# HoangGiang93/mujoco_sim

Measured on AMD Instinct MI355X. Metric: env-steps/sec (whole node) at 4096 envs, 24-DoF/30-contact scene; 1/2/4/8 GPUs, higher is better.
Workload: dtype f32

## Files before the change

mujoco_sim_amd/build.py:

```python
import os
import subprocess
import sys

HERE = os.path.dirname(os.path.abspath(__file__))
CSRC = os.path.join(HERE, "csrc")
OBJ = os.path.join(HERE, "build")
LIB = os.path.join(HERE, "libmjhip.so")
API = os.path.join("..", "..", "include", "mjhip.h")
KERNEL_HEADERS = ["step_kernel.h", "patch_pgs.h", "window_pgs.h", "dev_math.h", "dev_collide.h", "dev_convex.h", "dev_types.h"]
DENSE_HEADERS = ["dense_pgs.h"] + KERNEL_HEADERS
WINDOW_HEADERS = ["window_kernel.h", "step_kernel.h", "patch_pgs.h", "window_pgs.h", "dev_math.h", "dev_collide.h", "dev_convex.h", "dev_types.h"]
SOURCES = {
    "engine.hip": KERNEL_HEADERS + ["dev_ray.h", "ray_bvh.h", "dev_depth.h", "dev_scan.h", "dev_heightscan.h", "dev_render.h", "dev_light.h", "dev_texture.h", "ray_tables.h", API],
    "window.hip": WINDOW_HEADERS + [API],
    "dense.hip": DENSE_HEADERS + [API],
    "hfield.hip": KERNEL_HEADERS + [API],
    "ray.hip": ["dev_ray.h", "ray_bvh.h", API],
    "depth.hip": ["dev_depth.h", "dev_ray.h", "ray_bvh.h", API],
    "scan.hip": ["dev_scan.h", "dev_depth.h", "dev_ray.h", "ray_bvh.h", API],
    "heightscan.hip": ["dev_heightscan.h", "dev_scan.h", "dev_depth.h", "dev_ray.h", "ray_bvh.h", API],
    "render.hip": ["dev_render.h", "dev_depth.h", "dev_ray.h", "ray_bvh.h", API],
    "light.hip": ["dev_light.h", "dev_render.h", "dev_depth.h", "dev_ray.h", "ray_bvh.h", API],
    "texture.hip": ["dev_texture.h", "dev_render.h", "dev_depth.h", "dev_ray.h", "ray_bvh.h", API],
    "group.hip": ["host_pool.h", API],
    "model_builder.cpp": ["hmath.h", API],
    "scenes.cpp": ["hmath.h", API],
    "host_sim.cpp": ["host_sim.h", API],
    "mjcf_loader.cpp": ["hmath.h", API],
}
FLAGS = ["--offload-arch=gfx950", "-O3", "-std=c++17", "-fPIC", "-munsafe-fp-atomics", "-fno-slp-vectorize", "-Wno-unused-result"]
SOURCE_FLAGS = {"window.hip": ["-mllvm", "-pragma-unroll-threshold=200000"]}
FLAGS += os.environ.get("MJH_EXTRA_FLAGS", "").split()
if os.environ.get("MJH_BUILD_DIR"):
    OBJ = os.environ["MJH_BUILD_DIR"]; LIB = os.path.join(OBJ, "libmjhip.so")


def _digest(paths, extra=""):
    import hashlib
    h = hashlib.sha256(extra.encode())
    for p in paths:
        if os.path.exists(p):
            with open(p, "rb") as f:
                h.update(f.read())
    return h.hexdigest()


def build(force=False, verbose=False):
    hipcc = os.environ.get("HIPCC", "/opt/rocm/bin/hipcc")
    os.makedirs(OBJ, exist_ok=True)
    objs, digests, stale = [], [], []
    for src, deps in SOURCES.items():
        sp = os.path.join(CSRC, src)
        if not os.path.exists(sp):
            continue
        op = os.path.join(OBJ, os.path.splitext(src)[0] + ".o")
        sflags = FLAGS + SOURCE_FLAGS.get(src, [])
        dg = _digest([sp] + [os.path.join(CSRC, d) for d in deps], " ".join(sflags))
        stamp = op + ".sha256"
        have = open(stamp).read().strip() if os.path.exists(stamp) else ""
        if force or not os.path.exists(op) or have != dg:
            stale.append(([hipcc] + sflags + ["-c", sp, "-o", op], stamp, dg))
        objs.append(op); digests.append(dg)
    link_dg = _digest([], " ".join(digests))
    link_stamp = os.path.join(OBJ, "libmjhip.sha256")
    have = open(link_stamp).read().strip() if os.path.exists(link_stamp) else ""
    if not force and os.path.exists(LIB) and have == link_dg:
        return LIB
    from concurrent.futures import ThreadPoolExecutor

    def _compile(job):
        cmd, stamp, dg = job
        if verbose:
            print(" ".join(cmd), file=sys.stderr)
        subprocess.check_call(cmd)
        with open(stamp, "w") as f:
            f.write(dg)
    with ThreadPoolExecutor(max_workers=max(1, min(4, len(stale)))) as pool:
        for r in [pool.submit(_compile, j) for j in stale]:
            r.result()
    if force or not os.path.exists(LIB) or have != link_dg:
        cmd = [hipcc, "--offload-arch=gfx950", "-shared", "-fPIC"] + objs + ["-ldl", "-o", LIB]
        if verbose:
            print(" ".join(cmd), file=sys.stderr)
        subprocess.check_call(cmd)
# ... 15 lines not shown
```

mujoco_sim_amd/csrc/window_kernel.h:

```cpp
#pragma once
#include "step_kernel.h"

#ifdef WN_PROF_CLK
#define WN_STAT0(x) min((int)(((long long)__builtin_amdgcn_s_memtime() - wn_t0) >> 5) + 1, (1 << 22) - 1)
#else
#define WN_STAT0(x) (x)
#endif

#ifdef MJH_ASM_PROBE
#define WN_STATS(env, ncon, nefc, niter) S.stats[4 * env + 1] = nefc
#else
#define WN_STATS(env, ncon, nefc, niter) S.stats[4 * env] = WN_STAT0(ncon); S.stats[4 * env + 1] = nefc; S.stats[4 * env + 2] = niter
#endif

#ifdef WN_PROF_CLK
__shared__ long long wn_t0;
#endif

#define WN_BC8(M) M(0) M(1) M(2) M(3) M(4) M(5) M(6) M(7)
template <int NV> struct WnWin { float J[NV]; float4 A0, A1, A2, A3; float aref, R, nw, half; };

#define WN_ROR2(d, s0, s1, r0, m0, r1, m1) "v_add_f32_dpp " d ", " s0 ", " s0 " row_ror:" #r0 " row_mask:0xf bank_mask:" #m0 "\n\tv_add_f32_dpp " d ", " s1 ", " s1 " row_ror:" #r1 " row_mask:0xf bank_mask:" #m1 "\n\t"
DEV float wn_fold_tail(const float* z) {
  const int q = threadIdx.x & 15;
  const bool b1 = (q & 2) != 0, b0 = (q & 1) != 0;
  float w[2];
#pragma unroll
  for (int k = 0; k < 2; k++) {
    const float s = b1 ? z[k + 2] : z[k], o = b1 ? z[k] : z[k + 2];
    w[k] = s + __builtin_bit_cast(float, __builtin_amdgcn_update_dpp(0, __builtin_bit_cast(int, o), 0x4E, 0xf, 0xf, true));
  }
  const float s = b0 ? w[1] : w[0], o = b0 ? w[0] : w[1];
  return s + __builtin_bit_cast(float, __builtin_amdgcn_update_dpp(0, __builtin_bit_cast(int, o), 0xB1, 0xf, 0xf, true));
}
DEV void wn_fold_8to4(const float* y, float* z) {
  asm volatile(WN_ROR2("%0", "%4", "%8", 12, 0x5, 4, 0xa) WN_ROR2("%1", "%5", "%9", 12, 0x5, 4, 0xa) WN_ROR2("%2", "%6", "%10", 12, 0x5, 4, 0xa) WN_ROR2("%3", "%7", "%11", 12, 0x5, 4, 0xa)
               : "=&v"(z[0]), "=&v"(z[1]), "=&v"(z[2]), "=&v"(z[3]) : "v"(y[0]), "v"(y[1]), "v"(y[2]), "v"(y[3]), "v"(y[4]), "v"(y[5]), "v"(y[6]), "v"(y[7]));
}
DEV float wn_fold16(const float* x) {
  float y[8], z[4];
  asm volatile("s_nop 1\n\t"
               WN_ROR2("%0", "%8", "%16", 8, 0x3, 8, 0xc) WN_ROR2("%1", "%9", "%17", 8, 0x3, 8, 0xc) WN_ROR2("%2", "%10", "%18", 8, 0x3, 8, 0xc) WN_ROR2("%3", "%11", "%19", 8, 0x3, 8, 0xc)
               WN_ROR2("%4", "%12", "%20", 8, 0x3, 8, 0xc) WN_ROR2("%5", "%13", "%21", 8, 0x3, 8, 0xc) WN_ROR2("%6", "%14", "%22", 8, 0x3, 8, 0xc) WN_ROR2("%7", "%15", "%23", 8, 0x3, 8, 0xc)
               : "=&v"(y[0]), "=&v"(y[1]), "=&v"(y[2]), "=&v"(y[3]), "=&v"(y[4]), "=&v"(y[5]), "=&v"(y[6]), "=&v"(y[7])
               : "v"(x[0]), "v"(x[1]), "v"(x[2]), "v"(x[3]), "v"(x[4]), "v"(x[5]), "v"(x[6]), "v"(x[7]),
                 "v"(x[8]), "v"(x[9]), "v"(x[10]), "v"(x[11]), "v"(x[12]), "v"(x[13]), "v"(x[14]), "v"(x[15]));
  wn_fold_8to4(y, z);
  return wn_fold_tail(z);
}
#define WN_FOLD24_BODY \
    WN_ROR2("%[ya0]", "%[x16]", "%[x20]", 8, 0x3, 8, 0xc) WN_ROR2("%[ya1]", "%[x17]", "%[x21]", 8, 0x3, 8, 0xc) WN_ROR2("%[ya2]", "%[x18]", "%[x22]", 8, 0x3, 8, 0xc) WN_ROR2("%[ya3]", "%[x19]", "%[x23]", 8, 0x3, 8, 0xc) \
    WN_ROR2("%[ya0]", "%[ya0]", "%[ya2]", 12, 0x5, 4, 0xa) WN_ROR2("%[ya1]", "%[ya1]", "%[ya3]", 12, 0x5, 4, 0xa) \
    "v_cndmask_b32_e64 %[t0], %[z2], %[z0], %[m1]\n\t" "v_cndmask_b32_e64 %[t1], %[z3], %[z1], %[m1]\n\t" "v_cndmask_b32_e64 %[t2], %[z0], %[z2], %[m1]\n\t" \
    "v_cndmask_b32_e64 %[t3], %[z1], %[z3], %[m1]\n\t" "v_cndmask_b32_e64 %[ya2], %[ya1], %[ya0], %[m1]\n\t" "v_cndmask_b32_e64 %[ya3], %[ya0], %[ya1], %[m1]\n\t"
// ... 195 lines not shown
  if (dl_lane && q < M.njnt) {
    const int qadr = jnt_qposadr[q], da = jnt_dofadr[q];
    float p[7];
#pragma unroll
    for (int k = 0; k < 7; k++) p[k] = bad ? S.initial_qpos[qrow + qadr + k] : wb[WN_QPOS + qadr + k];
    const float* v = s_v32[es] + da;
    p[0] += h * v[0]; p[1] += h * v[1]; p[2] += h * v[2];
    float w3[3] = {v[3], v[4], v[5]};
    quat_integrate(p + 3, w3, h);
#pragma unroll
    for (int k = 0; k < 7; k++) { S.qpos[qrow + qadr + k] = p[k]; s_qp32[es][qadr + k] = p[k]; }
  }
  if (has_odom) {
    __syncthreads();
    if (dl_lane && q == 0) wn_odom(M, S, env, s_qp32[es], S.qvel + vrow);
  }
  if (dl_lane && q == 0) {
    S.time[env] += M.timestep_d;
    const int cost_hint = wn_cost_hint(M, nwin16, niter);
    WN_STATS(env, wh[1], wh[2], niter);
    S.stats[4 * env + 3] = ((S.stats[4 * env + 3] | flags) & 0xff) | (cost_hint << 8);
  }
}

DEV void wn_run32(const DConst* __restrict__ C, const DState& S, const int env0, const int nenv, const int xflags, const int blk) {
  const DModel& M = C->M;
  constexpr int NV = 24;
  const int lane = threadIdx.x, es = lane >> 5, hq = (lane >> 4) & 1, q = lane & 15;
  const int slot = blk * 2 + es;
  const bool have = slot < nenv;
  const int env = have ? (S.env_order ? S.env_order[env0 + slot] : env0 + slot) : 0;
  float* const wb = S.wbuf + (size_t)env * (size_t)S.wstride;
  const int* const wh = (const int*)wb;
  const int nrow = (have && wh[4] == 1) ? wh[0] : 0;
  if (__ballot(nrow > 0) == 0ull) return;
  const bool mine = nrow > 0;
  const int nwin16 = (nrow + 15) >> 4, nwin = (nrow + 31) >> 5;
  const int nwmax = max(__builtin_amdgcn_readlane(nwin, 0), __builtin_amdgcn_readlane(nwin, 32));
  const int nv = M.nv;
  const int dhi = 16 + (q >> 1);
  const bool lo_on = q < nv, hi_on = dhi < nv;
  const float as_lo = lo_on ? wb[WN_AS + q] : 0.0f, as_hi = hi_on ? wb[WN_AS + dhi] : 0.0f;
  const float ws_lo = lo_on ? wb[WN_AWS + q] : 0.0f, ws_hi = hi_on ? wb[WN_AWS + dhi] : 0.0f;
  WnWin32 win[WN32_NW];
  float f[WN32_NW];
  const float* rows = wb + WN_ROWS + q;
#pragma unroll
  for (int w = 0; w < WN32_NW; w++) if (w < nwmax) {
    WnWin32& W = win[w];
    const bool ok = (2 * w + hq) < nwin16;
    wn_load_row<NV>(rows + (2 * w + hq) * WN_NK * 16, ok, W.J, W.aref, W.R);
    float acc[16], acx[16], Jx[NV];
#pragma unroll
    for (int sidx = 0; sidx < 16; sidx++) { acc[sidx] = 0.0f; acx[sidx] = 0.0f; }
#pragma unroll
    for (int k = 0; k < NV; k++) Jx[k] = WN_SWZ16(W.J[k]);
#pragma unroll
    for (int k = 0; k < NV; k++) asm volatile("" : "+v"(W.J[k]), "+v"(Jx[k]));
    asm volatile("s_nop 1");
#define WN_ACC(sidx) PP_FMAC_BC(acc[sidx], W.J[k], W.J[k], sidx); PP_FMAC_BC(acx[sidx], Jx[k], W.J[k], sidx);
#pragma unroll
    for (int k = 0; k < NV; k++) { PP_BC16(WN_ACC) }
#undef WN_ACC
    float diag = 0.0f;
#pragma unroll
    for (int k = 0; k < NV; k++) diag += W.J[k] * W.J[k];
    const float ARqq = diag + W.R;
    const float inv = ARqq < MJ_MINVAL ? 0.0f : 1.0f / ARqq, ninv = -inv, cinv = hq ? ninv : 0.0f;
    W.nw = ninv; W.half = 0.5f * ARqq;
    W.A0 = make_float4(0 < q ? ninv * acc[0] : 0.0f, 1 < q ? ninv * acc[1] : 0.0f, 2 < q ? ninv * acc[2] : 0.0f, 3 < q ? ninv * acc[3] : 0.0f);
    W.A1 = make_float4(4 < q ? ninv * acc[4] : 0.0f, 5 < q ? ninv * acc[5] : 0.0f, 6 < q ? ninv * acc[6] : 0.0f, 7 < q ? ninv * acc[7] : 0.0f);
    W.A2 = make_float4(8 < q ? ninv * acc[8] : 0.0f, 9 < q ? ninv * acc[9] : 0.0f, 10 < q ? ninv * acc[10] : 0.0f, 11 < q ? ninv * acc[11] : 0.0f);
    W.A3 = make_float4(12 < q ? ninv * acc[12] : 0.0f, 13 < q ? ninv * acc[13] : 0.0f, 14 < q ? ninv * acc[14] : 0.0f, 0.0f);
    W.C0 = make_float4(cinv * acx[0], cinv * acx[1], cinv * acx[2], cinv * acx[3]);
    W.C1 = make_float4(cinv * acx[4], cinv * acx[5], cinv * acx[6], cinv * acx[7]);
    W.C2 = make_float4(cinv * acx[8], cinv * acx[9], cinv * acx[10], cinv * acx[11]);
    W.C3 = make_float4(cinv * acx[12], cinv * acx[13], cinv * acx[14], cinv * acx[15]);
  }
  auto rowsum_i32 = [&](int v) __attribute__((always_inline)) { v = wn_rowsum_i(v); return v + __builtin_amdgcn_ds_swizzle(v, 0x401F); };
  auto rowsum_f32 = [&](float v) __attribute__((always_inline)) { v = wn_rowsum_f(v); return v + WN_SWZ16(v); };
#define WN32_FOR_WINDOWS(...) do { _Pragma("unroll") for (int w = 0; w < WN32_NW; w++) if (w < nwmax) { WnWin32& W = win[w]; float& fw = f[w]; __VA_ARGS__ } } while (0)
  float a_lo = as_lo, a_hi = as_hi;
#pragma unroll
  for (int w = 0; w < WN32_NW; w++) f[w] = 0.0f;
  if (!(M.disableflags & MJH_DSBL_WARMSTART)) {
    float da_lo = 0.0f, da_hi = 0.0f;
    WN32_FOR_WINDOWS({
      const float jar = wn_dot<NV>(W.J, ws_lo, ws_hi) - W.aref;
      fw = (jar < 0.0f && W.R > 0.0f) ? -jar / W.R : 0.0f;
      wn_jt32(W.J, fw, da_lo, da_hi);
    });
    float cost = 0.0f;
    WN32_FOR_WINDOWS({
      const float jda = wn_dot<NV>(W.J, da_lo, da_hi), bb = wn_dot<NV>(W.J, as_lo, as_hi) - W.aref;
      cost += fw * (0.5f * (jda + W.R * fw) + bb);
    });
    cost = rowsum_f32(cost);
    if (cost > 0.0f) {
#pragma unroll
      for (int w = 0; w < WN32_NW; w++) f[w] = 0.0f;
    } else { a_lo += da_lo; a_hi += da_hi; }
  }
  const ImpQ iq = imp_quantum(1.0f / (M.meaninertia * (float)(nv > 1 ? nv : 1)), M.tolerance);
  const int itmax = M.iterations;
  int niter = 0;
  bool act = nrow > 0;
  while (__ballot(act) != 0ull) {
    if (act) {
      int impl = 0;
      WN32_FOR_WINDOWS({
        const float u = wn_dot<NV, false>(W.J, a_lo, a_hi);
        const float fo = fw;
        float tt = ((u - W.aref) + W.R * fo) * W.nw;
        const float nf = -fo;
        float dl;
        WN_ROWS4M(0, 1, 2, 3, W.A0, 0x5); WN_ROWS4M(4, 5, 6, 7, W.A1, 0x5); WN_ROWS4M(8, 9, 10, 11, W.A2, 0x5); WN_ROWS4M(12, 13, 14, 15, W.A3, 0x5);
// ... 106 lines not shown
    WN64_CHAIN16F(W.A, 16, 0x2, 0, 0xc, dx0);                    \
    WN64_BCAST_X1(W.A, 16, 0x4);                                 \
    dx1 = dy; \
    WN64_CHAIN16F(W.A, 32, 0x4, 16, 0x8, dx1);                   \
    WN64_BCAST_X2(W.A, 32, 0x8); \
    WN64_CHAIN16(W.A, 48, 0x8); \
    impl += imp_fixed((W.half * dl) * (2.0f * tt - dl), iq.qs); \
    fw = fo + dl; \
    wn_jt64(W.J, dl, a_lo, a_hi); } while (0)
#ifndef WN_FILL64
#define WN_FILL64 1
#endif
#if WN_FILL64
#define WN64_SWEEP(W, fw) WN64_SWEEP_F(W, fw)
#else
#define WN64_SWEEP(W, fw) WN64_SWEEP_X(W, fw, W.A, 0, 16, 32, 48, (void)0, (void)0, (void)0, (void)0)
#endif

template <int N64W, int N64T> DEV void wn_run64(const DConst* __restrict__ C, const DState& S, const int env0, const int nenv, const int xflags, const int blk, float* const lds64) {
  const DModel& M = C->M;
  constexpr int NV = 24;
  const int lane = threadIdx.x, g = lane >> 4, q = lane & 15;
  const bool have = blk < nenv;
  const int env = have ? (S.env_order ? S.env_order[env0 + blk] : env0 + blk) : 0;
  float* const wb = S.wbuf + (size_t)env * (size_t)S.wstride;
  const int* const wh = (const int*)wb;
  const int nrow = (have && wh[4] == 2) ? wh[0] : 0;
  if (nrow <= 0) return;
  const int nwin16 = (nrow + 15) >> 4, nwin = (nrow + 63) >> 6;
  const int nv = M.nv;
  const int dhi = 16 + (q >> 1);
  const bool lo_on = q < nv, hi_on = dhi < nv;
  const float as_lo = lo_on ? wb[WN_AS + q] : 0.0f, as_hi = hi_on ? wb[WN_AS + dhi] : 0.0f;
  const float ws_lo = lo_on ? wb[WN_AWS + q] : 0.0f, ws_hi = hi_on ? wb[WN_AWS + dhi] : 0.0f;
  WnWin64 win[N64W];
  float f[N64W];
  const float* rows = wb + WN_ROWS + q;
#pragma unroll
  for (int w = 0; w < N64W; w++) if (w < nwin) {
    WnWin64& W = win[w];
    const bool ok = (4 * w + g) < nwin16;
    wn_load_row<NV>(rows + (4 * w + g) * WN_NK * 16, ok, W.J, W.aref, W.R);
    float diag = 0.0f;
#pragma unroll
    for (int k = 0; k < NV; k++) diag += W.J[k] * W.J[k];
    const float ARqq = diag + W.R;
    const float inv = ARqq < MJ_MINVAL ? 0.0f : 1.0f / ARqq, ninv = -inv;
    W.nw = ninv; W.half = 0.5f * ARqq;
#pragma unroll
    for (int G = 0; G < 4; G++) {
      float Jg[NV], acc[16];
#pragma unroll
      for (int k = 0; k < NV; k++) Jg[k] = __builtin_bit_cast(float, __builtin_amdgcn_ds_bpermute((16 * G + q) << 2, __builtin_bit_cast(int, W.J[k])));
#pragma unroll
      for (int sidx = 0; sidx < 16; sidx++) acc[sidx] = 0.0f;
#pragma unroll
      for (int k = 0; k < NV; k++) asm volatile("" : "+v"(W.J[k]), "+v"(Jg[k]));
      asm volatile("s_nop 1");
#define WN_ACC(sidx) PP_FMAC_BC(acc[sidx], Jg[k], W.J[k], sidx);
#pragma unroll
      for (int k = 0; k < NV; k++) { PP_BC16(WN_ACC) }
#undef WN_ACC
#pragma unroll
      for (int sidx = 0; sidx < 16; sidx++) W.A[16 * G + sidx] = (16 * G + sidx) < lane ? ninv * acc[sidx] : 0.0f;
    }
  }
  struct WnTail { float J[NV]; float aref, R, nw, half; };
  WnTail TLS[N64T > 0 ? N64T : 1];
  float ftl[N64T > 0 ? N64T : 1];
  float* const tile = lds64 + lane * 4;
#pragma unroll
  for (int t = 0; t < N64T; t++) {
    ftl[t] = 0.0f;
    if (N64W + t < nwin) {
    WnTail& TL = TLS[t];
    const bool ok = (4 * (N64W + t) + g) < nwin16;
    wn_load_row<NV>(rows + (4 * (N64W + t) + g) * WN_NK * 16, ok, TL.J, TL.aref, TL.R);
    float diag = 0.0f;
#pragma unroll
    for (int k = 0; k < NV; k++) diag += TL.J[k] * TL.J[k];
    const float ARqq = diag + TL.R;
    const float inv = ARqq < MJ_MINVAL ? 0.0f : 1.0f / ARqq, ninv = -inv;
    TL.nw = ninv; TL.half = 0.5f * ARqq;
#pragma unroll
    for (int G = 0; G < 4; G++) {
      float Jg[NV], acc[16];
#pragma unroll
      for (int k = 0; k < NV; k++) Jg[k] = __builtin_bit_cast(float, __builtin_amdgcn_ds_bpermute((16 * G + q) << 2, __builtin_bit_cast(int, TL.J[k])));
#pragma unroll
      for (int sidx = 0; sidx < 16; sidx++) acc[sidx] = 0.0f;
#pragma unroll
      for (int k = 0; k < NV; k++) asm volatile("" : "+v"(TL.J[k]), "+v"(Jg[k]));
      asm volatile("s_nop 1");
#define WN_ACC(sidx) PP_FMAC_BC(acc[sidx], Jg[k], TL.J[k], sidx);
#pragma unroll
      for (int k = 0; k < NV; k++) { PP_BC16(WN_ACC) }
#undef WN_ACC
#pragma unroll
      for (int c4 = 0; c4 < 4; c4++) {
        const int r0 = 16 * G + 4 * c4;
        *(float4*)(tile + t * 4096 + (r0 >> 2) * 256) = make_float4(r0 < lane ? ninv * acc[4 * c4] : 0.0f, r0 + 1 < lane ? ninv * acc[4 * c4 + 1] : 0.0f,
                                                                    r0 + 2 < lane ? ninv * acc[4 * c4 + 2] : 0.0f, r0 + 3 < lane ? ninv * acc[4 * c4 + 3] : 0.0f);
      }
    }
    }
  }
  float T[16];
#define WN64_TLOAD(t, gb) do { const float* tp_ = tile + (t) * 4096 + (4 * (gb)) * 256; \
    const float4 t0_ = *(const float4*)(tp_), t1_ = *(const float4*)(tp_ + 256), t2_ = *(const float4*)(tp_ + 512), t3_ = *(const float4*)(tp_ + 768); \
    T[0] = t0_.x; T[1] = t0_.y; T[2] = t0_.z; T[3] = t0_.w; T[4] = t1_.x; T[5] = t1_.y; T[6] = t1_.z; T[7] = t1_.w; \
    T[8] = t2_.x; T[9] = t2_.y; T[10] = t2_.z; T[11] = t2_.w; T[12] = t3_.x; T[13] = t3_.y; T[14] = t3_.z; T[15] = t3_.w; } while (0)
#define WN64_FOR_TAILS(...) do { _Pragma("unroll") for (int t = 0; t < N64T; t++) if (N64W + t < nwin) { WnTail& TL = TLS[t]; float& ft = ftl[t]; __VA_ARGS__ } } while (0)
  float a_lo = as_lo, a_hi = as_hi;
#pragma unroll
  for (int w = 0; w < N64W; w++) f[w] = 0.0f;
#define WN64_FOR_WINDOWS(...) do { _Pragma("unroll") for (int w = 0; w < N64W; w++) if (w < nwin) { WnWin64& W = win[w]; float& fw = f[w]; __VA_ARGS__ } } while (0)
  if (!(M.disableflags & MJH_DSBL_WARMSTART)) {
    float da_lo = 0.0f, da_hi = 0.0f;
    WN64_FOR_WINDOWS({
      const float jar = wn_dot<NV>(W.J, ws_lo, ws_hi) - W.aref;
      fw = (jar < 0.0f && W.R > 0.0f) ? -jar / W.R : 0.0f;
      wn_jt64(W.J, fw, da_lo, da_hi);
    });
    WN64_FOR_TAILS({
      const float jar = wn_dot<NV>(TL.J, ws_lo, ws_hi) - TL.aref;
      ft = (jar < 0.0f && TL.R > 0.0f) ? -jar / TL.R : 0.0f;
      wn_jt64(TL.J, ft, da_lo, da_hi);
    });
    float cost = 0.0f;
    WN64_FOR_WINDOWS({
      const float jda = wn_dot<NV>(W.J, da_lo, da_hi), bb = wn_dot<NV>(W.J, as_lo, as_hi) - W.aref;
      cost += fw * (0.5f * (jda + W.R * fw) + bb);
    });
    WN64_FOR_TAILS({
      const float jda = wn_dot<NV>(TL.J, da_lo, da_hi), bb = wn_dot<NV>(TL.J, as_lo, as_hi) - TL.aref;
      cost += ft * (0.5f * (jda + TL.R * ft) + bb);
    });
    float dummy = 0.0f;
    cost = wn_rowsum_f(cost); wn_rows4_sum2(cost, dummy);
    if (cost > 0.0f) {
#pragma unroll
      for (int w = 0; w < N64W; w++) f[w] = 0.0f;
#pragma unroll
      for (int t = 0; t < N64T; t++) ftl[t] = 0.0f;
    } else { a_lo += da_lo; a_hi += da_hi; }
  }
  const ImpQ iq = imp_quantum(1.0f / (M.meaninertia * (float)(nv > 1 ? nv : 1)), M.tolerance);
  const int itmax = M.iterations;
  int niter = 0;
  while (true) {
// ... 54 lines not shown
      [j0] "v"(WN_J2(JA, 0)), [j1] "v"(WN_J2(JA, 1)), [j2] "v"(WN_J2(JA, 2)), [j3] "v"(WN_J2(JA, 3)), [j4] "v"(WN_J2(JA, 4)), [j5] "v"(WN_J2(JA, 5)), [j6] "v"(WN_J2(JA, 6)), [j7] "v"(WN_J2(JA, 7)))
#define WN_ROWS8_FB1(T0, T1, P, JA) asm volatile( \
    WN_ROWF(8, "%[a0]", WN_FPK("%[p0]", "%[j0]")) WN_ROWF(9, "%[a1]", WN_FPK("%[p1]", "%[j1]")) WN_ROWF(10, "%[a2]", WN_FPK("%[p2]", "%[j2]")) WN_ROWF(11, "%[a3]", WN_FPK("%[p3]", "%[j3]")) \
    WN_ROWF(12, "%[a4]", "v_mul_f32 %[e1], %[hf], %[da]") WN_ROWF(13, "%[a5]", "v_fma_f32 %[e2], 2.0, %[ta], -%[da]") WN_ROWF(14, "%[a6]", "v_mul_f32 %[e1], %[e1], %[e2]") WN_ROWF(15, "%[a7]", "v_mul_f32 %[e1], %[e1], %[qs]") \
    "v_max_f32 %[d], %[t], %[nf]" \
    : [t] "+v"(tt), [d] "=&v"(dl), [p0] "=&v"(P[8]), [p1] "=&v"(P[9]), [p2] "=&v"(P[10]), [p3] "=&v"(P[11]), [e1] "=&v"(e1), [e2] "=&v"(e2) \
    : [nf] "v"(nf), [x2] "v"(xa2), [a0] "v"(T0.x), [a1] "v"(T0.y), [a2] "v"(T0.z), [a3] "v"(T0.w), [a4] "v"(T1.x), [a5] "v"(T1.y), [a6] "v"(T1.z), [a7] "v"(T1.w), \
      [j0] "v"(WN_J2(JA, 8)), [j1] "v"(WN_J2(JA, 9)), [j2] "v"(WN_J2(JA, 10)), [j3] "v"(WN_J2(JA, 11)), [hf] "v"(A.half), [da] "v"(dla), [ta] "v"(tta), [qs] "v"(iq.qs))

#ifndef WN_X_LDS
#define WN_X_LDS 1
#endif
#ifndef WN_STRAIGHT
#define WN_STRAIGHT 1
#endif
#define WN_XLDS_BYTES(nvt, nw) (((nvt) == 24 && WN_FILL && WN_X_LDS) ? ((nw) / 2) * 4 * 64 * 16 : 0)
template <int NV, int NW, bool XL = false, int N64W = WN64_NW, int N64T = WN64_NT>
__global__ __launch_bounds__(64, 1) void mjh_window_kernel(const DConst* __restrict__ C, const DState S, const int env0, const int nenv, const int nl, const int xflags, const int n32waves, const int n64waves) {
#ifdef WN_PROF_CLK
  if (threadIdx.x == 0) wn_t0 = (long long)__builtin_amdgcn_s_memtime();
  __syncthreads();
#endif
  if constexpr (NV == 24) {
#ifndef WN_NO_F64
    if ((int)blockIdx.x < n64waves) { wn_run64<N64W, N64T>(C, S, env0, nenv, xflags, (int)blockIdx.x, wn_lds_base()); return; }
#endif
    if ((int)blockIdx.x < n64waves + n32waves) { wn_run32(C, S, env0, nenv, xflags, (int)blockIdx.x - n64waves); return; }
  }
  const DModel& M = C->M;
  const int lane = threadIdx.x, rho = lane >> 4, q = lane & 15;
  const int slot = ((int)blockIdx.x - n32waves - n64waves) * 4 + rho;
  const bool have = slot < nenv;
  const int env = have ? (S.env_order ? S.env_order[env0 + slot] : env0 + slot) : 0;
  float* const wb = S.wbuf + (size_t)env * (size_t)S.wstride;
  const int* const wh = (const int*)wb;
  const int nrow = (have && !(n32waves > 0 && wh[4] == 1) && !(n64waves > 0 && wh[4] == 2)) ? wh[0] : 0;
  const bool mine = nrow > 0 || (have && wh[5] == 1);
  if (__ballot(mine) == 0ull) return;
  const int nwin = (nrow + 15) >> 4;
  const int nwmax = max(max(__builtin_amdgcn_readlane(nwin, 0), __builtin_amdgcn_readlane(nwin, 16)), max(__builtin_amdgcn_readlane(nwin, 32), __builtin_amdgcn_readlane(nwin, 48)));
  const int nv = M.nv;
  const int dhi = NV == 24 ? 16 + (q >> 1) : 16 + q;
  const bool lo_on = q < nv, hi_on = dhi < nv;
  const float as_lo = lo_on ? wb[WN_AS + q] : 0.0f, as_hi = hi_on ? wb[WN_AS + dhi] : 0.0f;
  const float ws_lo = lo_on ? wb[WN_AWS + q] : 0.0f, ws_hi = hi_on ? wb[WN_AWS + dhi] : 0.0f;

  WnWin<NV> win[NW];
  float f[NW];
  const float* rows = wb + WN_ROWS + q;
  auto load_rows = [&](WnWin<NV>& W, const int w) __attribute__((always_inline)) {
    const bool ok = w < nwin;
    wn_load_row<NV>(rows + w * WN_NK * 16, ok, W.J, W.aref, W.R);
  };
  auto make_tile = [&](WnWin<NV>& W) __attribute__((always_inline)) {
    float acc[16];
#pragma unroll
    for (int s = 0; s < 16; s++) acc[s] = 0.0f;
#pragma unroll
    for (int k = 0; k < NV; k++) asm volatile("" : "+v"(W.J[k]));
    asm volatile("s_nop 1");
#define WN_ACC(s) PP_FMAC_BC(acc[s], W.J[k], W.J[k], s);
#pragma unroll
    for (int k = 0; k < NV; k++) { PP_BC16(WN_ACC) }
#undef WN_ACC
    float diag = 0.0f;
#pragma unroll
    for (int k = 0; k < NV; k++) diag += W.J[k] * W.J[k];
    const float ARqq = diag + W.R;
    const float inv = ARqq < MJ_MINVAL ? 0.0f : 1.0f / ARqq, ninv = -inv;
    W.nw = ninv; W.half = 0.5f * ARqq;
    W.A0 = make_float4(0 < q ? ninv * acc[0] : 0.0f, 1 < q ? ninv * acc[1] : 0.0f, 2 < q ? ninv * acc[2] : 0.0f, 3 < q ? ninv * acc[3] : 0.0f);
    W.A1 = make_float4(4 < q ? ninv * acc[4] : 0.0f, 5 < q ? ninv * acc[5] : 0.0f, 6 < q ? ninv * acc[6] : 0.0f, 7 < q ? ninv * acc[7] : 0.0f);
    W.A2 = make_float4(8 < q ? ninv * acc[8] : 0.0f, 9 < q ? ninv * acc[9] : 0.0f, 10 < q ? ninv * acc[10] : 0.0f, 11 < q ? ninv * acc[11] : 0.0f);
    W.A3 = make_float4(12 < q ? ninv * acc[12] : 0.0f, 13 < q ? ninv * acc[13] : 0.0f, 14 < q ? ninv * acc[14] : 0.0f, 0.0f);
  };
  constexpr int NX4 = WN_XREC(NV) / 4, NJ4 = NV / 4;
  static_assert(NV % 4 == 0 && NX4 == NJ4 + 6, "window record layout");
  auto store_ext = [&](float4* t, const WnWin<NV>& W, const float fw) __attribute__((always_inline)) {
#pragma unroll
    for (int k = 0; k < NJ4; k++) t[16 * k] = make_float4(W.J[4 * k], W.J[4 * k + 1], W.J[4 * k + 2], W.J[4 * k + 3]);
    t[16 * NJ4] = W.A0; t[16 * (NJ4 + 1)] = W.A1; t[16 * (NJ4 + 2)] = W.A2; t[16 * (NJ4 + 3)] = W.A3;
    t[16 * (NJ4 + 4)] = make_float4(W.aref, W.R, W.nw, W.half);
    *(float*)(t + 16 * (NJ4 + 5)) = fw;
  };
  auto load_ext = [&](const float4* t, WnWin<NV>& W) __attribute__((always_inline)) {
#pragma unroll
    for (int k = 0; k < NJ4; k++) { const float4 j = t[16 * k]; W.J[4 * k] = j.x; W.J[4 * k + 1] = j.y; W.J[4 * k + 2] = j.z; W.J[4 * k + 3] = j.w; }
    W.A0 = t[16 * NJ4]; W.A1 = t[16 * (NJ4 + 1)]; W.A2 = t[16 * (NJ4 + 2)]; W.A3 = t[16 * (NJ4 + 3)];
    const float4 c = t[16 * (NJ4 + 4)];
    W.aref = c.x; W.R = c.y; W.nw = c.z; W.half = c.w;
  };
#define WN_XF(t) (*(float*)((t) + 16 * (NJ4 + 5)))
  float4* const xl = (float4*)wn_lds + (rho * nl * NX4) * 16 + q;
  float4* const xg = (float4*)(wb + WN_ROWS + M.win_maxw * WN_NK * 16) + q;
  const int nwl = min(nwmax, NW + nl);
#pragma unroll
  for (int w = 0; w < NW; w++) if (w < nwmax) { load_rows(win[w], w); make_tile(win[w]); }
  static_assert(NW % 2 == 0, "register-resident windows are swept in pairs");
  float4 X[NW / 2][4];
  auto make_cross = [&](WnWin<NV>& A, WnWin<NV>& B, float4 (&Xo)[4]) __attribute__((always_inline)) {
    float acx[16];
#pragma unroll
    for (int sidx = 0; sidx < 16; sidx++) acx[sidx] = 0.0f;
#pragma unroll
    for (int k = 0; k < NV; k++) asm volatile("" : "+v"(A.J[k]), "+v"(B.J[k]));
    asm volatile("s_nop 1");
#define WN_ACX(sidx) PP_FMAC_BC(acx[sidx], A.J[k], B.J[k], sidx);
#pragma unroll
    for (int k = 0; k < NV; k++) { PP_BC16(WN_ACX) }
#undef WN_ACX
    Xo[0] = make_float4(B.nw * acx[0], B.nw * acx[1], B.nw * acx[2], B.nw * acx[3]);
    Xo[1] = make_float4(B.nw * acx[4], B.nw * acx[5], B.nw * acx[6], B.nw * acx[7]);
    Xo[2] = make_float4(B.nw * acx[8], B.nw * acx[9], B.nw * acx[10], B.nw * acx[11]);
    Xo[3] = make_float4(B.nw * acx[12], B.nw * acx[13], B.nw * acx[14], B.nw * acx[15]);
  };
  constexpr bool X_LDS = XL && NV == 24 && WN_FILL && WN_X_LDS;
  float4* const xs = (float4*)wn_lds + (4 * nl * NX4) * 16 + lane;
#pragma unroll
  for (int j = 0; j < NW / 2; j++) if (2 * j + 1 < nwmax) {
    make_cross(win[2 * j], win[2 * j + 1], X[j]);
    if constexpr (X_LDS) {
#pragma unroll
      for (int c = 0; c < 4; c++) xs[(4 * j + c) * 64] = X[j][c];
    }
  }
  for (int w = NW; w < nwl; w++) { WnWin<NV> W; load_rows(W, w); make_tile(W); store_ext(xl + (w - NW) * NX4 * 16, W, 0.0f); }
  for (int w = nwl; w < nwmax; w++) { WnWin<NV> W; load_rows(W, w); make_tile(W); if (mine) store_ext(xg + w * NX4 * 16, W, 0.0f); }
  auto load_tier = [&](const int w, WnWin<NV>& W, float& fw) __attribute__((always_inline)) {
    if (w < nwl) { const float4* t = xl + (w - NW) * NX4 * 16; load_ext(t, W); fw = WN_XF(t); }
    else {
      const float4* t = xg + w * NX4 * 16; fw = 0.0f;
      if (mine) { load_ext(t, W); fw = WN_XF(t); } else { load_rows(W, WN_MAXW); W.A0 = W.A1 = W.A2 = W.A3 = make_float4(0, 0, 0, 0); W.nw = 0; W.half = 0; }
    }
  };
  auto store_tier_force = [&](const int w, const float fw) __attribute__((always_inline)) {
    if (w < nwl) WN_XF(xl + (w - NW) * NX4 * 16) = fw; else if (mine) WN_XF(xg + w * NX4 * 16) = fw;
  };
  constexpr bool TIER_PAIRS = NV == 24 && WN_FILL && WN_TIER_PAIRS;
  float4* const xx = xg + M.win_maxw * NX4 * 16;
  if constexpr (TIER_PAIRS) for (int w = NW; w + 1 < nwmax; w += 2) {
    WnWin<NV> A, B; float fdum; float4 Xo[4];
    load_tier(w, A, fdum); load_tier(w + 1, B, fdum);
    make_cross(A, B, Xo);
    if (mine) { float4* tx = xx + ((w - NW) >> 1) * 64; tx[0] = Xo[0]; tx[16] = Xo[1]; tx[32] = Xo[2]; tx[48] = Xo[3]; }
  }
#define WN_FOR_WINDOWS(...) do { \
    _Pragma("unroll") for (int w = 0; w < NW; w++) if (w < nwmax) { WnWin<NV>& W = win[w]; float& fw = f[w]; __VA_ARGS__ } \
    for (int w = NW; w < nwl; w++) { WnWin<NV> W; float4* t = xl + (w - NW) * NX4 * 16; load_ext(t, W); float fw = WN_XF(t); __VA_ARGS__ WN_XF(t) = fw; } \
    for (int w = nwl; w < nwmax; w++) { WnWin<NV> W; float4* t = xg + w * NX4 * 16; float fw = 0.0f; if (mine) { load_ext(t, W); fw = WN_XF(t); } else { load_rows(W, WN_MAXW); W.A0 = W.A1 = W.A2 = W.A3 = make_float4(0, 0, 0, 0); W.nw = 0; W.half = 0; } \
                                          __VA_ARGS__ if (mine) WN_XF(t) = fw; } } while (0)
#define WN_ZERO_EXT_FORCES() do { for (int w = NW; w < nwl; w++) WN_XF(xl + (w - NW) * NX4 * 16) = 0.0f; \
                                  if (mine) for (int w = nwl; w < nwmax; w++) WN_XF(xg + w * NX4 * 16) = 0.0f; } while (0)

  float a_lo = as_lo, a_hi = as_hi;
#pragma unroll
  for (int w = 0; w < NW; w++) f[w] = 0.0f;
  if (!(M.disableflags & MJH_DSBL_WARMSTART)) {
    float da_lo = 0.0f, da_hi = 0.0f;
    WN_FOR_WINDOWS({
      const float jar = wn_dot<NV>(W.J, ws_lo, ws_hi) - W.aref;
      fw = (jar < 0.0f && W.R > 0.0f) ? -jar / W.R : 0.0f;
      wn_jt<NV>(W.J, fw, da_lo, da_hi);
    });
    float cost = 0.0f;
    WN_FOR_WINDOWS({
      const float jda = wn_dot<NV>(W.J, da_lo, da_hi), bb = wn_dot<NV>(W.J, as_lo, as_hi) - W.aref;
      cost += fw * (0.5f * (jda + W.R * fw) + bb);
    });
    cost = wn_rowsum_f(cost);
    if (cost > 0.0f) {
#pragma unroll
      for (int w = 0; w < NW; w++) f[w] = 0.0f;
      WN_ZERO_EXT_FORCES();
    } else { a_lo += da_lo; a_hi += da_hi; }
  }
  const ImpQ iq = imp_quantum(1.0f / (M.meaninertia * (float)(nv > 1 ? nv : 1)), M.tolerance);
  const int itmax = M.iterations;
// ... 217 lines not shown
```

Baseline: 16.47 million.

## Compute window Gram tiles with MFMA 16x16x1 instead of DPP broadcast FMAs

Adds a window_tiles.h helper that builds the 16x16 J·Jᵀ tiles with chained mfma_f32_16x16x1f32 instructions and then permutes the accumulator back into the per-lane layout using permlane32/16 swaps. The DPP-broadcast FMA path is kept as a fallback. In the register-resident prologue, the self tiles of both windows in a pair and their cross tile now run as three interleaved MFMA chains. It also enables the -amdgpu-mfma-vgpr-form build flag. The goal is to move the VALU-heavy tile construction onto the matrix cores, at the cost of extra permute instructions and possible register pressure from the 16-wide accumulators.

```diff
diff --git a/mujoco_sim_amd/build.py b/mujoco_sim_amd/build.py
--- a/mujoco_sim_amd/build.py
+++ b/mujoco_sim_amd/build.py
@@ -9,7 +9,7 @@
 API = os.path.join("..", "..", "include", "mjhip.h")
 KERNEL_HEADERS = ["step_kernel.h", "patch_pgs.h", "window_pgs.h", "dev_math.h", "dev_collide.h", "dev_convex.h", "dev_types.h"]
 DENSE_HEADERS = ["dense_pgs.h"] + KERNEL_HEADERS
-WINDOW_HEADERS = ["window_kernel.h", "step_kernel.h", "patch_pgs.h", "window_pgs.h", "dev_math.h", "dev_collide.h", "dev_convex.h", "dev_types.h"]
+WINDOW_HEADERS = ["window_kernel.h", "window_tiles.h", "step_kernel.h", "patch_pgs.h", "window_pgs.h", "dev_math.h", "dev_collide.h", "dev_convex.h", "dev_types.h"]
 SOURCES = {
     "engine.hip": KERNEL_HEADERS + ["dev_ray.h", "ray_bvh.h", "dev_depth.h", "dev_scan.h", "dev_heightscan.h", "dev_render.h", "dev_light.h", "dev_texture.h", "ray_tables.h", API],
     "window.hip": WINDOW_HEADERS + [API],
@@ -29,7 +29,7 @@
     "mjcf_loader.cpp": ["hmath.h", API],
 }
 FLAGS = ["--offload-arch=gfx950", "-O3", "-std=c++17", "-fPIC", "-munsafe-fp-atomics", "-fno-slp-vectorize", "-Wno-unused-result"]
-SOURCE_FLAGS = {"window.hip": ["-mllvm", "-pragma-unroll-threshold=200000"]}
+SOURCE_FLAGS = {"window.hip": ["-mllvm", "-pragma-unroll-threshold=200000", "-mllvm", "-amdgpu-mfma-vgpr-form"]}
 FLAGS += os.environ.get("MJH_EXTRA_FLAGS", "").split()
 if os.environ.get("MJH_BUILD_DIR"):
     OBJ = os.environ["MJH_BUILD_DIR"]; LIB = os.path.join(OBJ, "libmjhip.so")
diff --git a/mujoco_sim_amd/csrc/window_kernel.h b/mujoco_sim_amd/csrc/window_kernel.h
--- a/mujoco_sim_amd/csrc/window_kernel.h
+++ b/mujoco_sim_amd/csrc/window_kernel.h
@@ -1,5 +1,6 @@
 #pragma once
 #include "step_kernel.h"
+#include "window_tiles.h"
 
 #ifdef WN_PROF_CLK
 #define WN_STAT0(x) min((int)(((long long)__builtin_amdgcn_s_memtime() - wn_t0) >> 5) + 1, (1 << 22) - 1)
@@ -301,16 +302,8 @@
     wn_load_row<NV>(rows + (2 * w + hq) * WN_NK * 16, ok, W.J, W.aref, W.R);
     float acc[16], acx[16], Jx[NV];
 #pragma unroll
-    for (int sidx = 0; sidx < 16; sidx++) { acc[sidx] = 0.0f; acx[sidx] = 0.0f; }
-#pragma unroll
     for (int k = 0; k < NV; k++) Jx[k] = WN_SWZ16(W.J[k]);
-#pragma unroll
-    for (int k = 0; k < NV; k++) asm volatile("" : "+v"(W.J[k]), "+v"(Jx[k]));
-    asm volatile("s_nop 1");
-#define WN_ACC(sidx) PP_FMAC_BC(acc[sidx], W.J[k], W.J[k], sidx); PP_FMAC_BC(acx[sidx], Jx[k], W.J[k], sidx);
-#pragma unroll
-    for (int k = 0; k < NV; k++) { PP_BC16(WN_ACC) }
-#undef WN_ACC
+    wn_tile16<NV>(W.J, W.J, acc); wn_tile16<NV>(Jx, W.J, acx);
     float diag = 0.0f;
 #pragma unroll
     for (int k = 0; k < NV; k++) diag += W.J[k] * W.J[k];
@@ -523,15 +516,7 @@
       float Jg[NV], acc[16];
 #pragma unroll
       for (int k = 0; k < NV; k++) Jg[k] = __builtin_bit_cast(float, __builtin_amdgcn_ds_bpermute((16 * G + q) << 2, __builtin_bit_cast(int, W.J[k])));
-#pragma unroll
-      for (int sidx = 0; sidx < 16; sidx++) acc[sidx] = 0.0f;
-#pragma unroll
-      for (int k = 0; k < NV; k++) asm volatile("" : "+v"(W.J[k]), "+v"(Jg[k]));
-      asm volatile("s_nop 1");
-#define WN_ACC(sidx) PP_FMAC_BC(acc[sidx], Jg[k], W.J[k], sidx);
-#pragma unroll
-      for (int k = 0; k < NV; k++) { PP_BC16(WN_ACC) }
-#undef WN_ACC
+      wn_tile16<NV>(Jg, W.J, acc);
 #pragma unroll
       for (int sidx = 0; sidx < 16; sidx++) W.A[16 * G + sidx] = (16 * G + sidx) < lane ? ninv * acc[sidx] : 0.0f;
     }
@@ -558,15 +543,7 @@
       float Jg[NV], acc[16];
 #pragma unroll
       for (int k = 0; k < NV; k++) Jg[k] = __builtin_bit_cast(float, __builtin_amdgcn_ds_bpermute((16 * G + q) << 2, __builtin_bit_cast(int, TL.J[k])));
-#pragma unroll
-      for (int sidx = 0; sidx < 16; sidx++) acc[sidx] = 0.0f;
-#pragma unroll
-      for (int k = 0; k < NV; k++) asm volatile("" : "+v"(TL.J[k]), "+v"(Jg[k]));
-      asm volatile("s_nop 1");
-#define WN_ACC(sidx) PP_FMAC_BC(acc[sidx], Jg[k], TL.J[k], sidx);
-#pragma unroll
-      for (int k = 0; k < NV; k++) { PP_BC16(WN_ACC) }
-#undef WN_ACC
+      wn_tile16<NV>(Jg, TL.J, acc);
 #pragma unroll
       for (int c4 = 0; c4 < 4; c4++) {
         const int r0 = 16 * G + 4 * c4;
@@ -727,17 +704,8 @@
     const bool ok = w < nwin;
     wn_load_row<NV>(rows + w * WN_NK * 16, ok, W.J, W.aref, W.R);
   };
-  auto make_tile = [&](WnWin<NV>& W) __attribute__((always_inline)) {
-    float acc[16];
-#pragma unroll
-    for (int s = 0; s < 16; s++) acc[s] = 0.0f;
-#pragma unroll
-    for (int k = 0; k < NV; k++) asm volatile("" : "+v"(W.J[k]));
-    asm volatile("s_nop 1");
-#define WN_ACC(s) PP_FMAC_BC(acc[s], W.J[k], W.J[k], s);
-#pragma unroll
-    for (int k = 0; k < NV; k++) { PP_BC16(WN_ACC) }
-#undef WN_ACC
+  constexpr bool TILE_MMA = WN_TILE_MFMA && NV == 24;
+  auto finish_tile = [&](WnWin<NV>& W, const float (&acc)[16]) __attribute__((always_inline)) {
     float diag = 0.0f;
 #pragma unroll
     for (int k = 0; k < NV; k++) diag += W.J[k] * W.J[k];
@@ -749,6 +717,11 @@
     W.A2 = make_float4(8 < q ? ninv * acc[8] : 0.0f, 9 < q ? ninv * acc[9] : 0.0f, 10 < q ? ninv * acc[10] : 0.0f, 11 < q ? ninv * acc[11] : 0.0f);
     W.A3 = make_float4(12 < q ? ninv * acc[12] : 0.0f, 13 < q ? ninv * acc[13] : 0.0f, 14 < q ? ninv * acc[14] : 0.0f, 0.0f);
   };
+  auto make_tile = [&](WnWin<NV>& W) __attribute__((always_inline)) {
+    float acc[16];
+    wn_tile16<NV, TILE_MMA>(W.J, W.J, acc);
+    finish_tile(W, acc);
+  };
   constexpr int NX4 = WN_XREC(NV) / 4, NJ4 = NV / 4;
   static_assert(NV % 4 == 0 && NX4 == NJ4 + 6, "window record layout");
   auto store_ext = [&](float4* t, const WnWin<NV>& W, const float fw) __attribute__((always_inline)) {
@@ -769,35 +742,34 @@
   float4* const xl = (float4*)wn_lds + (rho * nl * NX4) * 16 + q;
   float4* const xg = (float4*)(wb + WN_ROWS + M.win_maxw * WN_NK * 16) + q;
   const int nwl = min(nwmax, NW + nl);
-#pragma unroll
-  for (int w = 0; w < NW; w++) if (w < nwmax) { load_rows(win[w], w); make_tile(win[w]); }
   static_assert(NW % 2 == 0, "register-resident windows are swept in pairs");
   float4 X[NW / 2][4];
-  auto make_cross = [&](WnWin<NV>& A, WnWin<NV>& B, float4 (&Xo)[4]) __attribute__((always_inline)) {
-    float acx[16];
-#pragma unroll
-    for (int sidx = 0; sidx < 16; sidx++) acx[sidx] = 0.0f;
-#pragma unroll
-    for (int k = 0; k < NV; k++) asm volatile("" : "+v"(A.J[k]), "+v"(B.J[k]));
-    asm volatile("s_nop 1");
-#define WN_ACX(sidx) PP_FMAC_BC(acx[sidx], A.J[k], B.J[k], sidx);
-#pragma unroll
-    for (int k = 0; k < NV; k++) { PP_BC16(WN_ACX) }
-#undef WN_ACX
+  auto finish_cross = [&](const WnWin<NV>& B, const float (&acx)[16], float4 (&Xo)[4]) __attribute__((always_inline)) {
     Xo[0] = make_float4(B.nw * acx[0], B.nw * acx[1], B.nw * acx[2], B.nw * acx[3]);
     Xo[1] = make_float4(B.nw * acx[4], B.nw * acx[5], B.nw * acx[6], B.nw * acx[7]);
     Xo[2] = make_float4(B.nw * acx[8], B.nw * acx[9], B.nw * acx[10], B.nw * acx[11]);
     Xo[3] = make_float4(B.nw * acx[12], B.nw * acx[13], B.nw * acx[14], B.nw * acx[15]);
   };
+  auto make_cross = [&](WnWin<NV>& A, WnWin<NV>& B, float4 (&Xo)[4]) __attribute__((always_inline)) {
+    float acx[16];
+    wn_tile16<NV, TILE_MMA>(A.J, B.J, acx);
+    finish_cross(B, acx, Xo);
+  };
   constexpr bool X_LDS = XL && NV == 24 && WN_FILL && WN_X_LDS;
   float4* const xs = (float4*)wn_lds + (4 * nl * NX4) * 16 + lane;
 #pragma unroll
-  for (int j = 0; j < NW / 2; j++) if (2 * j + 1 < nwmax) {
-    make_cross(win[2 * j], win[2 * j + 1], X[j]);
-    if constexpr (X_LDS) {
-#pragma unroll
-      for (int c = 0; c < 4; c++) xs[(4 * j + c) * 64] = X[j][c];
-    }
+  for (int j = 0; j < NW / 2; j++) {
+    if (2 * j + 1 < nwmax) {
+      WnWin<NV>& A = win[2 * j]; WnWin<NV>& B = win[2 * j + 1];
+      load_rows(A, 2 * j); load_rows(B, 2 * j + 1);
+      float acca[16], accb[16], acx[16];
+      wn_tile16_pair<NV, TILE_MMA>(A.J, B.J, acca, accb, acx);
+      finish_tile(A, acca); finish_tile(B, accb); finish_cross(B, acx, X[j]);
+      if constexpr (X_LDS) {
+#pragma unroll
+        for (int c = 0; c < 4; c++) xs[(4 * j + c) * 64] = X[j][c];
+      }
+    } else if (2 * j < nwmax) { load_rows(win[2 * j], 2 * j); make_tile(win[2 * j]); }
   }
   for (int w = NW; w < nwl; w++) { WnWin<NV> W; load_rows(W, w); make_tile(W); store_ext(xl + (w - NW) * NX4 * 16, W, 0.0f); }
   for (int w = nwl; w < nwmax; w++) { WnWin<NV> W; load_rows(W, w); make_tile(W); if (mine) store_ext(xg + w * NX4 * 16, W, 0.0f); }
diff --git a/mujoco_sim_amd/csrc/window_tiles.h b/mujoco_sim_amd/csrc/window_tiles.h
--- /dev/null
+++ b/mujoco_sim_amd/csrc/window_tiles.h
@@ -0,0 +1,80 @@
+#pragma once
+
+#ifndef WN_TILE_MFMA
+#define WN_TILE_MFMA 1
+#endif
+
+#ifndef WN_TILE_CHAINS
+#define WN_TILE_CHAINS 3
+#endif
+
+typedef float wn_f32x16 __attribute__((ext_vector_type(16)));
+
+template <int NK> __device__ __forceinline__ wn_f32x16 wn_tile16_mma(const float* A, const float* B) {
+  wn_f32x16 d = {0.0f, 0.0f, 0.0f, 0.0f, 0.0f, 0.0f, 0.0f, 0.0f, 0.0f, 0.0f, 0.0f, 0.0f, 0.0f, 0.0f, 0.0f, 0.0f};
+#pragma unroll
+  for (int k = 0; k < NK; k++) d = __builtin_amdgcn_mfma_f32_16x16x1f32(A[k], B[k], d, 0, 0, 0);
+  return d;
+}
+
+__device__ __forceinline__ void wn_tile16_home(const wn_f32x16 d, float* acc) {
+  unsigned r[16];
+#pragma unroll
+  for (int i = 0; i < 16; i++) { const float x = d[i]; r[i] = __builtin_bit_cast(unsigned, x); }
+#pragma unroll
+  for (int i = 0; i < 8; i++) {
+    const auto p = __builtin_amdgcn_permlane32_swap(r[i], r[i + 8], false, false);
+    r[i] = p[0]; r[i + 8] = p[1];
+  }
+#pragma unroll
+  for (int i = 0; i < 16; i++) if (!(i & 4)) {
+    const auto p = __builtin_amdgcn_permlane16_swap(r[i], r[i + 4], false, false);
+    r[i] = p[0]; r[i + 4] = p[1];
+  }
+#pragma unroll
+  for (int i = 0; i < 16; i++) acc[i] = __builtin_bit_cast(float, r[i]);
+}
+
+#define WN_TILE_FMAC_BC(acc, x, y, R) asm volatile("v_fmac_f32_dpp %0, %1, %2 row_newbcast:" #R " row_mask:0xf bank_mask:0xf" : "+v"(acc) : "v"(x), "v"(y))
+#define WN_TILE_BC16(M) M(0) M(1) M(2) M(3) M(4) M(5) M(6) M(7) M(8) M(9) M(10) M(11) M(12) M(13) M(14) M(15)
+template <int NK> __device__ __forceinline__ void wn_tile16_bcast(float* A, float* B, float* acc) {
+#pragma unroll
+  for (int s = 0; s < 16; s++) acc[s] = 0.0f;
+#pragma unroll
+  for (int k = 0; k < NK; k++) asm volatile("" : "+v"(A[k]));
+  if (A != B) {
+#pragma unroll
+    for (int k = 0; k < NK; k++) asm volatile("" : "+v"(B[k]));
+  }
+  asm volatile("s_nop 1");
+#define WN_TILE_ACC(s) WN_TILE_FMAC_BC(acc[s], A[k], B[k], s);
+#pragma unroll
+  for (int k = 0; k < NK; k++) { WN_TILE_BC16(WN_TILE_ACC) }
+#undef WN_TILE_ACC
+}
+
+template <int NK, bool MFMA = (WN_TILE_MFMA != 0)> __device__ __forceinline__ void wn_tile16(float* A, float* B, float* acc) {
+  if constexpr (MFMA) wn_tile16_home(wn_tile16_mma<NK>(A, B), acc);
+  else wn_tile16_bcast<NK>(A, B, acc);
+}
+
+template <int NK, bool MFMA = (WN_TILE_MFMA != 0)> __device__ __forceinline__ void wn_tile16_pair(float* U, float* V, float* accU, float* accV, float* accX) {
+  if constexpr (MFMA && WN_TILE_CHAINS == 1) {
+    wn_tile16<NK, true>(U, U, accU); __builtin_amdgcn_sched_barrier(0);
+    wn_tile16<NK, true>(V, V, accV); __builtin_amdgcn_sched_barrier(0);
+    wn_tile16<NK, true>(U, V, accX);
+  } else if constexpr (MFMA) {
+    wn_f32x16 du, dv, dx;
+#pragma unroll
+    for (int i = 0; i < 16; i++) { du[i] = 0.0f; dv[i] = 0.0f; dx[i] = 0.0f; }
+#pragma unroll
+    for (int k = 0; k < NK; k++) {
+      du = __builtin_amdgcn_mfma_f32_16x16x1f32(U[k], U[k], du, 0, 0, 0);
+      dv = __builtin_amdgcn_mfma_f32_16x16x1f32(V[k], V[k], dv, 0, 0, 0);
+      dx = __builtin_amdgcn_mfma_f32_16x16x1f32(U[k], V[k], dx, 0, 0, 0);
+    }
+    wn_tile16_home(du, accU); wn_tile16_home(dv, accV); wn_tile16_home(dx, accX);
+  } else {
+    wn_tile16_bcast<NK>(U, U, accU); wn_tile16_bcast<NK>(V, V, accV); wn_tile16_bcast<NK>(U, V, accX);
+  }
+}
```

New measurement: 16.69 million, median of 6. 1.01x the previous value.
